# itmo153277/JoshUpscale

Hardware: AMD Instinct MI355X
Metric: frames/sec 480x270->1920x1080 recurrent SR (higher is better)
Workload: dtype bf16

## Files before the change

joshupscale_amd/csrc/tower_kernels.hip:

```cpp
#include "kernel_common.h"

namespace ju {

namespace {

constexpr int kTowerThreads = 256;
constexpr int kTowerWBytes = 9 * 64 * 64 * 2;
constexpr int kTowerTileBytes = 10 * 34 * 128;
constexpr int kTowerLds = kTowerWBytes + 2 * kTowerTileBytes;

__device__ __forceinline__ void glds16(const void *g, void *l) {
	__builtin_amdgcn_global_load_lds((const __attribute__((address_space(1))) void *)g,
	    (__attribute__((address_space(3))) void *)l, 16, 0, 0);
}

struct TowerParams {
	const void *in;
	const void *wgt;
	const float *bias;
	const void *res;
	void *out;
	int H, W, pitch;
	int tilesX, numTiles;
	int relu;
// ... 35 lines not shown
		}
	};

	{
		const unsigned char *wsrc = static_cast<const unsigned char *>(p.wgt);
#pragma unroll
		for (int k = 0; k < (VARIANT == 4 ? 0 : 18); ++k) {
			const int i = wave + 4 * k;
			glds16(wsrc + (size_t)i * 1024 + lane * 16, smW + i * 1024);
		}
	}
	int tile = slot;
	if (tile < p.numTiles) stageTile(tile, 0);

	f32x4 biasv[2][4];
#pragma unroll
	for (int nb = 0; nb < 2; ++nb) {
#pragma unroll
		for (int g = 0; g < 4; ++g) {
			biasv[nb][g] = *reinterpret_cast<const f32x4 *>(p.bias + nb * 32 + 8 * g + 4 * hh);
		}
	}
	asm volatile("s_waitcnt vmcnt(0)" ::: "memory");
	__syncthreads();

	const unsigned ldsBase = static_cast<unsigned>(reinterpret_cast<unsigned long long>(
	    (__attribute__((address_space(3))) unsigned char *)smem));
	const unsigned wAddr = ldsBase + hh * 1024 + px * 16;
	const unsigned wAddrHi = wAddr + 40960;
	const int q0 = (wave * 2) * 34 + px;

	int buf = 0;
	const int stride = perX * 8;
	for (; tile < p.numTiles; tile += stride, buf ^= 1) {
		const int next = tile + stride;
		if (next < p.numTiles) stageTile(next, buf ^ 1);

		const int ty = tile / p.tilesX;
		const int tx = tile - ty * p.tilesX;
		f32x16 acc[2][2];
#pragma unroll
		for (int nb = 0; nb < 2; ++nb) {
#pragma unroll
			for (int g = 0; g < 4; ++g) {
#pragma unroll
				for (int rw = 0; rw < 2; ++rw) {
					acc[nb][rw][4 * g + 0] = biasv[nb][g][0];
					acc[nb][rw][4 * g + 1] = biasv[nb][g][1];
					acc[nb][rw][4 * g + 2] = biasv[nb][g][2];
					acc[nb][rw][4 * g + 3] = biasv[nb][g][3];
				}
			}
		}
		Vec4<T> resv[2][2][4];
		if (VARIANT != 2 && p.res != nullptr) {
			const int gxr = tx * 32 + px;
#pragma unroll
			for (int rw = 0; rw < 2; ++rw) {
				const int gyr = ty * 8 + wave * 2 + rw;
				const T *rp = static_cast<const T *>(p.res) +
				              ((size_t)(gyr + 1) * p.pitch + gxr + 1) * 64 + 4 * hh;
#pragma unroll
				for (int nb = 0; nb < 2; ++nb) {
#pragma unroll
					for (int g = 0; g < 4; ++g) {
						resv[rw][nb][g] = *reinterpret_cast<const Vec4<T> *>(rp + nb * 32 + 8 * g);
					}
				}
			}
		}

		Vec8<T> fa[2][3][2], fb[2][4];
		const unsigned tileAddr = ldsBase + kTowerWBytes + buf * kTowerTileBytes;
		auto issueRead = [&](int m, int set, int idx) {
			const int dx = m >> 2, ks = m & 3;
			constexpr int kind[10] = {0, 1, 0, 1, 0, 0, 1, 0, 0, 1};
			constexpr int sub[10] = {0, 0, 1, 1, 2, 3, 2, 4, 5, 3};
			if (kind[idx] == 0) {
				const int dy = sub[idx] >> 1, nb = sub[idx] & 1;
				const int widx = (dy * 3 + dx) * 4 + ks;
				const int off = widx * 2048 + nb * 512;
				if (off < 65536 - 512) {
					asm volatile("ds_read_b128 %0, %1 offset:%2"
					             : "=v"(fa[set][dy][nb]) : "v"(wAddr), "n"(off));
				} else {
					asm volatile("ds_read_b128 %0, %1 offset:%2"
					             : "=v"(fa[set][dy][nb]) : "v"(wAddrHi), "n"(off - 40960));
				}
			} else {
				const int r = sub[idx];
				const int q = q0 + r * 34 + dx;
				const unsigned a = tileAddr + q * 128 + (((ks * 2 + hh) ^ ((q >> 1) & 7)) << 4);
				asm volatile("ds_read_b128 %0, %1" : "=v"(fb[set][r]) : "v"(a));
			}
		};
		constexpr int needs[12] = {1, 2, 3, -1, 4, 5, 6, -1, 7, 8, 9, -1};
		asm volatile("s_waitcnt lgkmcnt(0)" ::: "memory");
		__builtin_amdgcn_sched_barrier(0);
#pragma unroll
		for (int i = 0; i < (VARIANT == 1 ? 0 : 10); ++i) issueRead(0, 0, i);
#pragma unroll
		for (int m = 0; m < (VARIANT == 1 ? 0 : 12); ++m) {
			const int set = m & 1;
			const bool more = (m + 1 < 12);
#pragma unroll
			for (int k = 0; k < 12; ++k) {
				if (needs[k] >= 0) {
					const int allowed = (9 - needs[k]) + (more ? (k < 10 ? k : 10) : 0);
					if (allowed >= 10) asm volatile("s_waitcnt lgkmcnt(10)" ::: "memory");
					else if (allowed == 9) asm volatile("s_waitcnt lgkmcnt(9)" ::: "memory");
					else if (allowed == 8) asm volatile("s_waitcnt lgkmcnt(8)" ::: "memory");
					else if (allowed == 7) asm volatile("s_waitcnt lgkmcnt(7)" ::: "memory");
					else if (allowed == 6) asm volatile("s_waitcnt lgkmcnt(6)" ::: "memory");
					else if (allowed == 5) asm volatile("s_waitcnt lgkmcnt(5)" ::: "memory");
					else if (allowed == 4) asm volatile("s_waitcnt lgkmcnt(4)" ::: "memory");
					else if (allowed == 3) asm volatile("s_waitcnt lgkmcnt(3)" ::: "memory");
					else if (allowed == 2) asm volatile("s_waitcnt lgkmcnt(2)" ::: "memory");
					else if (allowed == 1) asm volatile("s_waitcnt lgkmcnt(1)" ::: "memory");
					else asm volatile("s_waitcnt lgkmcnt(0)" ::: "memory");
					__builtin_amdgcn_sched_barrier(0);
				}
				const int dy = k >> 2, rw = (k >> 1) & 1, nb = k & 1;
				acc[nb][rw] = mfma32(fa[set][dy][nb], fb[set][rw + dy], acc[nb][rw]);
				if (more && k < 10) issueRead(m + 1, set ^ 1, k);
				__builtin_amdgcn_sched_barrier(0);
			}
		}
		asm volatile("s_waitcnt vmcnt(0)" ::: "memory");
		__syncthreads();
		{
			unsigned char *slice = smT + buf * kTowerTileBytes + wave * 8192;
#pragma unroll
			for (int rw = 0; rw < 2; ++rw) {
				const int pi = rw * 32 + px;
#pragma unroll
				for (int nb = 0; nb < 2; ++nb) {
#pragma unroll
					for (int g = 0; g < 4; ++g) {
						float v[4];
#pragma unroll
						for (int i = 0; i < 4; ++i) v[i] = acc[nb][rw][4 * g + i];
						if (VARIANT != 2 && p.res != nullptr) {
#pragma unroll
							for (int i = 0; i < 4; ++i) v[i] += static_cast<float>(resv[rw][nb][g][i]);
						}
						if (p.relu == 1) {
#pragma unroll
							for (int i = 0; i < 4; ++i) v[i] = fmaxf(v[i], 0.0f);
						} else if (p.relu == 2) {
#pragma unroll
							for (int i = 0; i < 4; ++i) v[i] = leaky(v[i], p.slope);
						}
						Vec4<T> o = {static_cast<T>(v[0]), static_cast<T>(v[1]),
						    static_cast<T>(v[2]), static_cast<T>(v[3])};
						const int c = nb * 4 + g;
						*reinterpret_cast<Vec4<T> *>(
						    slice + pi * 128 + ((c ^ (pi & 7)) << 4) + hh * 8) = o;
					}
				}
			}
			__builtin_amdgcn_fence(__ATOMIC_RELEASE, "wavefront");
			__builtin_amdgcn_wave_barrier();
			__builtin_amdgcn_fence(__ATOMIC_ACQUIRE, "wavefront");
			if (VARIANT != 2) {
				T *outp = static_cast<T *>(p.out);
#pragma unroll
				for (int i = 0; i < 8; ++i) {
					const int pi = i * 8 + (lane >> 3);
					const int c = (lane & 7) ^ (pi & 7);
					typedef unsigned u32x4 __attribute__((ext_vector_type(4)));
					const u32x4 val = *reinterpret_cast<const u32x4 *>(slice + i * 1024 + lane * 16);
					const int gy = ty * 8 + wave * 2 + (pi >> 5);
					const int gxo = tx * 32 + (pi & 31);
					if (gy < p.H && gxo < p.W) {
						*reinterpret_cast<u32x4 *>(
						    outp + ((size_t)(gy + 1) * p.pitch + gxo + 1) * 64 + c * 8) = val;
					}
				}
			} else {
				asm volatile("" ::"v"(acc[0][0]), "v"(acc[1][0]), "v"(acc[0][1]), "v"(acc[1][1]));
			}
		}
		asm volatile("s_waitcnt lgkmcnt(0)" ::: "memory");
		__builtin_amdgcn_s_barrier();
		__builtin_amdgcn_sched_barrier(0);
	}
}

int g_TowerVariant = 0;
int g_ResidentFault = 0;

template <typename T, int VARIANT>
void launchTowerT(const ConvParams &p, hipStream_t stream) {
	auto kern = conv_tower_kernel<T, VARIANT>;
	static std::atomic<std::uint64_t> ldsDone{0};
	ensureDynamicLds(reinterpret_cast<const void *>(kern), kTowerLds, &ldsDone, "tower");
	const int pitch = towerPitch(p.W);
	const size_t origin = towerOrigin(p.W) * 64 * 2;
	TowerParams t{};
	t.in = static_cast<const unsigned char *>(p.in) - origin;
	t.wgt = p.wgt;
	t.bias = p.bias;
	t.res = p.res ? static_cast<const unsigned char *>(p.res) - origin : nullptr;
	t.out = static_cast<unsigned char *>(p.out) - origin;
	t.H = p.H;
	t.W = p.W;
	t.pitch = pitch;
	t.tilesX = (p.W + 31) / 32;
	t.numTiles = t.tilesX * ((p.H + 7) / 8);
	t.relu = p.relu;
	t.slope = p.slope;
	const int grid = ((t.numTiles < 256 ? t.numTiles : 256) + 7) / 8 * 8;
	hipLaunchKernelGGL(kern, dim3(grid), dim3(kTowerThreads), kTowerLds, stream, t);
	hipCheckLaunch("conv_tower");
}

#ifndef JU_TOWER_M16
#define JU_TOWER_M16 1
#endif
#if JU_TOWER_M16
struct TowerAcc {
	f32x4 q[4];
};
__device__ __forceinline__ float accElem(const TowerAcc &a, const int i) { return a.q[i >> 2][i & 3]; }
__device__ __forceinline__ void setAccElem(TowerAcc &a, const int i, const float v) { a.q[i >> 2][i & 3] = v; }
#else
typedef f32x16 TowerAcc;
__device__ __forceinline__ float accElem(const TowerAcc &a, const int i) { return a[i]; }
__device__ __forceinline__ void setAccElem(TowerAcc &a, const int i, const float v) { a[i] = v; }
#endif
constexpr int kResRW = 32;
constexpr int kResMaxRH = 16;
constexpr int kResPitch = kResRW + 2;
constexpr int kResRowBytes = kResPitch * 128;
constexpr int kResBufBytes = (kResMaxRH + 2) * kResRowBytes;
constexpr int kResDummyOff = kResBufBytes;
constexpr int kResOffA = 0;
constexpr int kResOffB = kResBufBytes + 16;
constexpr int kResOffMisc = kResOffB + kResBufBytes + 16;
static_assert(kResRowBytes == 4352, "the ds_read immediates in tower_resident_kernel assume a 4352-byte row");
constexpr int kResLds = kResOffMisc + 64 + 512;
constexpr int kResMailSlots = 4 * 32 * 8;
constexpr unsigned long long kResTimeoutTicks = 20000000ull;
#ifndef JU_PRERUN
#define JU_PRERUN 2
#endif
#ifndef JU_PREBEFORE
#define JU_PREBEFORE 1
#endif
#ifndef JU_FAST_PRERUN
#define JU_FAST_PRERUN 2
#endif

__host__ __device__ inline bool residentFastShape(int rhv, int rwv) {
	if ((rhv & 1) || rwv < 2) return false;
#if JU_TOWER_M16
	if (rwv != 32) return false;
#endif
	const int np2 = rhv >> 1;
	for (int par = 0; par < 2; ++par) {
		const int first = par ? 1 : 2;
		int n = 0;
		for (int k = 0; k < 2; ++k) {
			const int u = first + 2 * k;
			if (u < np2 && 2 * u + 3 <= rhv) n = k + 1;
		}
		const int mine = (np2 - par + 1) >> 1;
		if (n != 2 || (mine != 3 && mine != 4)) return false;
	}
	return true;
}

struct ResidentParams {
	const void *in;
	int inPitch;
	int hasHead;
	void *out;
	const void *weights;
	const float *bias;
	uint4 *mail;
	unsigned *count;
	unsigned *error;
	unsigned long long *debug;
	int H, W, pitch;
	int GX, GY, RH;
	int nLayers;
	float slope;
	const void *tailW1;
	const float *tailB1;
	const void *tailW2;
	const float *tailB2;
	const std::uint8_t *frame;
	std::ptrdiff_t frameStride;
	void *state;
	std::uint8_t *outU8;
	std::ptrdiff_t outStride;
	const unsigned *sums;
};

typedef unsigned long long u64;
typedef __attribute__((address_space(1))) u64 gu64;
typedef __attribute__((address_space(1))) unsigned gu32;

template <typename T, int VARIANT, bool HEAD, bool TAIL = false, bool LEAKY = false, bool FAST = false>
__global__ __launch_bounds__(256, 1) void tower_resident_kernel(ResidentParams p) {
	static_assert(!FAST || ((VARIANT == 0 || VARIANT == 4) && (JU_FAST_PRERUN == 2 || JU_FAST_PRERUN == 3)), "the fast schedule is built for the product only");
	extern __shared__ __attribute__((aligned(16))) unsigned char smem[];
	constexpr bool kNoMfma = VARIANT == 2 || VARIANT == 3;
#ifdef JU_NOXCHG_DEV
	constexpr bool xchg = false;
#else
	constexpr bool xchg = !(VARIANT == 1 || VARIANT == 3);
#endif
	const int tid = threadIdx.x;
	const int wave = tid >> 6;
	const int lane = tid & 63;
	const int px = lane & 31;
	const int hh = lane >> 5;
	const int ch = wave & 1;
	const int rp = wave >> 1;
	int region;
	{
		const int n = gridDim.x, x = blockIdx.x & 7;
		int start = 0;
		for (int y = 0; y < x; ++y) start += (n - y + 7) >> 3;
		region = start + (blockIdx.x >> 3);
	}
	const int gxr = region % p.GX;
	const int gyr = region / p.GX;
	const int x0 = gxr * kResRW;
	const int y0 = gyr * p.RH;
	const int rwv = min(kResRW, p.W - x0);
	const int rhv = min(p.RH, p.H - y0);
	volatile int *failFlag = reinterpret_cast<volatile int *>(smem + kResOffMisc);
	unsigned pubCount[2] = {p.count[region * 2], p.count[region * 2 + 1]};

	const unsigned ldsBase = static_cast<unsigned>(reinterpret_cast<unsigned long long>(
	    (__attribute__((address_space(3))) unsigned char *)smem));

	for (int i = tid; i < kResOffMisc / 16; i += 256) {
		reinterpret_cast<uint4 *>(smem)[i] = make_uint4(0, 0, 0, 0);
	}
	if (tid == 0) *failFlag = 0;
	__syncthreads();

	{
		const T *in = static_cast<const T *>(p.in);
		const int nPix = (rhv + 2) * kResPitch;
		const int nInstr = (nPix + 7) / 8;
		for (int i = wave; i < nInstr; i += 4) {
			const int q = i * 8 + (lane >> 3);
			const int rr = q / kResPitch, cc = q - rr * kResPitch;
			const int c = (lane & 7) ^ ((cc >> 1) & 7);
			const int gy = y0 - 1 + rr, gx = x0 - 1 + cc;
			if (q < nPix && gy >= 0 && gy < p.H && gx >= 0 && gx < p.W) {
				glds16(in + ((size_t)gy * p.inPitch + gx) * 64 + c * 8, smem + kResOffA + i * 1024);
			}
		}
	}

	typedef unsigned u32x4w __attribute__((ext_vector_type(4)));
	const __amdgpu_buffer_rsrc_t wRsrc = __builtin_amdgcn_make_buffer_rsrc(
	    const_cast<void *>(p.weights), 0, p.nLayers * 73728, 0x00020000);
#if JU_TOWER_M16
	const unsigned wLaneOff = (unsigned)((ch * 64 + lane) * 16);
#else
	const unsigned wLaneOff = (unsigned)((hh * 64 + ch * 32 + px) * 16);
#endif
	auto loadWeightFrag = [&](int layer, int f) __attribute__((always_inline)) -> Vec8<T> {
		const u32x4w v = __builtin_amdgcn_raw_buffer_load_b128(wRsrc, wLaneOff, layer * 73728 + f * 2048, 0);
		return __builtin_bit_cast(Vec8<T>, v);
	};
	Vec8<T> wm[12], ws[24];
	auto loadMidWeights = [&](int layer) __attribute__((always_inline)) {
#pragma unroll
		for (int f = 0; f < 36; ++f) {
			if ((f >> 2) % 3 == 1) wm[(f / 12) * 4 + (f & 3)] = loadWeightFrag(layer, f);
		}
	};
	auto loadSideWeights = [&](int layer) __attribute__((always_inline)) {
#pragma unroll
		for (int f = 0; f < 36; ++f) {
			const int dx = (f >> 2) % 3;
			if (dx != 1) ws[(f / 12) * 8 + (dx >> 1) * 4 + (f & 3)] = loadWeightFrag(layer, f);
		}
	};
	loadMidWeights(0);
	loadSideWeights(0);
	const __amdgpu_buffer_rsrc_t biasRsrc = __builtin_amdgcn_make_buffer_rsrc(
	    const_cast<float *>(p.bias), 0, p.nLayers * 256, 0x00020000);
	TowerAcc biasVec;
	auto loadBias = [&](int layer) __attribute__((always_inline)) {
#if JU_TOWER_M16
#pragma unroll
		for (int c16 = 0; c16 < 2; ++c16) {
			const u32x4w v = __builtin_amdgcn_raw_buffer_load_b128(biasRsrc, (unsigned)((ch * 32 + c16 * 16 + 4 * (lane >> 4)) * 4), layer * 256, 0);
#pragma unroll
			for (int i = 0; i < 4; ++i) {
				setAccElem(biasVec, 4 * c16 + i, __uint_as_float(v[i]));
				setAccElem(biasVec, 8 + 4 * c16 + i, __uint_as_float(v[i]));
			}
		}
#else
#pragma unroll
		for (int g = 0; g < 4; ++g) {
			const u32x4w v = __builtin_amdgcn_raw_buffer_load_b128(biasRsrc, (unsigned)((ch * 32 + 4 * hh + 8 * g) * 4), layer * 256, 0);
#pragma unroll
			for (int i = 0; i < 4; ++i) setAccElem(biasVec, 4 * g + i, __uint_as_float(v[i]));
		}
#endif
	};
	loadBias(0);

	unsigned colBase[3], colSwz[3];
#pragma unroll
	for (int dx = 0; dx < 3; ++dx) {
#if JU_TOWER_M16
		const int cq = (lane & 15) + dx;
#else
		const int cq = px + dx;
#endif
		colBase[dx] = cq * 128;
		colSwz[dx] = (cq >> 1) & 7;
	}
	unsigned outsw[4];
#pragma unroll
	for (int g = 0; g < 4; ++g) {
#if JU_TOWER_M16
		const int cq = (g >> 1) * 16 + (lane & 15) + 1;
		outsw[g] = cq * 128 + (((ch * 4 + (g & 1) * 2 + (lane >> 5)) ^ ((cq >> 1) & 7)) << 4) + ((lane >> 4) & 1) * 8;
#else
		const int cq = px + 1;
		outsw[g] = cq * 128 + (((ch * 4 + g) ^ ((cq >> 1) & 7)) << 4) + hh * 8;
#endif
	}

	asm volatile("s_waitcnt vmcnt(0)" ::: "memory");
	__syncthreads();

	u64 prof[8] = {0, 0, 0, 0, 0, 0, 0, 0};
	u64 extraPasses = 0;
	float calibMax = 0.f;
	auto stamp = [&]() __attribute__((always_inline)) -> u64 {
		if constexpr (VARIANT == 4) {
			__builtin_amdgcn_sched_barrier(0);
			u64 t;
			asm volatile("s_memtime %0\n\ts_waitcnt lgkmcnt(0)" : "=s"(t)::"memory");
			__builtin_amdgcn_sched_barrier(0);
			return t;
		} else {
			return 0;
		}
	};
	constexpr int kOrder[12] = {4, 5, 6, 7, 0, 1, 2, 3, 8, 9, 10, 11};
	constexpr bool kPlain = VARIANT == 8;
	constexpr int kPreRun = kPlain ? 0 : FAST ? JU_FAST_PRERUN : JU_PRERUN;
	constexpr int kPreBefore = kPlain ? 0 : JU_PREBEFORE;
	TowerAcc accPre0[2], accPre1[2], accPre2[2];
	static_assert(kPreRun >= 0 && kPreRun <= 3, "at most three interior units per wave");
	Vec8<T> fb[2][4];
	auto issue = [&](unsigned rowAddr, int m, int set, int j) __attribute__((always_inline)) {
#if JU_TOWER_M16
		const int dx = m >> 2, ks32 = (m >> 1) & 1, ph = m & 1;
		const unsigned a = rowAddr + colBase[dx] + (((unsigned)(ks32 * 4 + (lane >> 4)) ^ colSwz[dx]) << 4);
		if (ph) {
			if (j == 0) asm volatile("ds_read_b128 %0, %1 offset:2048" : "=v"(fb[set][0]) : "v"(a));
			else if (j == 1) asm volatile("ds_read_b128 %0, %1 offset:6400" : "=v"(fb[set][1]) : "v"(a));
			else if (j == 2) asm volatile("ds_read_b128 %0, %1 offset:10752" : "=v"(fb[set][2]) : "v"(a));
			else asm volatile("ds_read_b128 %0, %1 offset:15104" : "=v"(fb[set][3]) : "v"(a));
			return;
		}
#else
		const int dx = m >> 2, ks = m & 3;
		const unsigned a = rowAddr + colBase[dx] + (((unsigned)(ks * 2 + hh) ^ colSwz[dx]) << 4);
#endif
		if (j == 0) asm volatile("ds_read_b128 %0, %1" : "=v"(fb[set][0]) : "v"(a));
		else if (j == 1) asm volatile("ds_read_b128 %0, %1 offset:4352" : "=v"(fb[set][1]) : "v"(a));
		else if (j == 2) asm volatile("ds_read_b128 %0, %1 offset:8704" : "=v"(fb[set][2]) : "v"(a));
		else asm volatile("ds_read_b128 %0, %1 offset:13056" : "=v"(fb[set][3]) : "v"(a));
	};
	const int np2 = rhv >> 1;
	const bool mySingle = (rhv & 1) && rp == (np2 & 1);
	const int preFirst = rp ? 1 : 2;
	int nPre = 0;
#pragma unroll
	for (int k = 0; k < kPreRun; ++k) {
		const int u = preFirst + 2 * k;
		if (u < np2 && 2 * u + 3 <= rhv) nPre = k + 1;
	}
	if constexpr (FAST && kPreRun == 3) {
		const int mine = (np2 - rp + 1) >> 1;
		nPre = nPre < mine - 1 ? nPre : mine - 1;
	}
	const int preEnd = preFirst + 2 * nPre;
	auto isPre = [&](int u) __attribute__((always_inline)) { return u >= preFirst && u < preEnd; };
	auto nextWhole = [&](int u) __attribute__((always_inline)) {
		int v = u + 2;
		if (isPre(v)) v = preEnd;
		return v < np2 ? v : -1;
	};
	const int firstWhole = isPre(rp) ? (preEnd < np2 ? preEnd : -1) : (rp < np2 ? rp : -1);
	const bool streamsInUnit = (firstWhole >= 0 || mySingle) && !kNoMfma && !kPlain;
	constexpr bool kDefer = FAST;
	const bool deferShape = residentFastShape(rhv, rwv);
	if constexpr (FAST) {
		if (!deferShape) {
			if (tid == 0) __hip_atomic_store((gu32 *)p.error, 0x6f0u, __ATOMIC_RELAXED, __HIP_MEMORY_SCOPE_SYSTEM);
			return;
		}
	}

#if JU_TOWER_M16
	const bool validLo = (lane & 15) < rwv, validHi = 16 + (lane & 15) < rwv;
	auto groupValid = [&](const int g) __attribute__((always_inline)) { return FAST || ((g >> 1) ? validHi : validLo); };
#else
	const bool lanesValid = px < rwv;
	auto groupValid = [&](const int) __attribute__((always_inline)) { return lanesValid; };
#endif
	typedef unsigned u32x4 __attribute__((ext_vector_type(4)));
	const __amdgpu_buffer_rsrc_t mailRsrc = __builtin_amdgcn_make_buffer_rsrc(
	    (void *)p.mail, 0, (int)((size_t)p.GX * p.GY * 2 * (LEAKY ? 2 : 1) * kResMailSlots * 16), 0x00020000);
	constexpr int kSc1 = 16;
	Vec4<T> rvNext[2][4];
	auto epiValue = [&](auto resTag, const TowerAcc &a, const int g, const Vec4<T> &rv, float(&v)[4]) __attribute__((always_inline)) {
#pragma unroll
		for (int i = 0; i < 4; ++i) v[i] = accElem(a, 4 * g + i);
		if constexpr (decltype(resTag)::value) {
#pragma unroll
			for (int i = 0; i < 4; ++i) v[i] += static_cast<float>(rv[i]);
		}
		if constexpr (VARIANT == 5 && !LEAKY) {
			if (groupValid(g)) {
#pragma unroll
				for (int i = 0; i < 4; ++i) calibMax = fmaxf(calibMax, v[i]);
			}
		}
	};
	auto epiStore = [&](auto outTag, const int row, const int g, float(&v)[4]) __attribute__((always_inline)) {
		constexpr int outOff = decltype(outTag)::value;
		if constexpr (LEAKY) {
#pragma unroll
			for (int i = 0; i < 4; ++i) v[i] = fmaxf(v[i], v[i] * p.slope);
			if constexpr (VARIANT == 5) {
#pragma unroll
				for (int i = 0; i < 4; ++i) calibMax = fmaxf(calibMax, fabsf(v[i]));
			}
			*reinterpret_cast<Vec4<T> *>(smem + outOff + row * kResRowBytes + outsw[g]) = pack4<T>(v[0], v[1], v[2], v[3]);
		} else {
			*reinterpret_cast<Vec4<T> *>(smem + outOff + row * kResRowBytes + outsw[g]) =
			    reluPacked<T>(pack4<T>(v[0], v[1], v[2], v[3]));
		}
	};
	auto unitSeg = [&](auto rowsTag, auto kindTag, auto resTag, auto inTag, auto outTag, TowerAcc(&acc)[2],
	                   const int layer, const int unit, const bool primed, const int nextUnit,
	                   const bool nextFinish, auto streamTag, auto defTag, TowerAcc(&dacc)[2], const int dunit,
	                   auto epiTag) __attribute__((always_inline)) {
		constexpr bool streamNext = decltype(streamTag)::value;
		constexpr bool DEF = decltype(defTag)::value;
		constexpr bool EPI = decltype(epiTag)::value;
		constexpr int ROWS = decltype(rowsTag)::value;
		constexpr int KIND = decltype(kindTag)::value;
		constexpr bool residual = decltype(resTag)::value;
		constexpr int inOff = decltype(inTag)::value;
		constexpr int outOff = decltype(outTag)::value;
		constexpr int P0 = KIND == 1 ? 4 : 0;
		constexpr int P1 = KIND == 0 ? 4 : 12;
		const u64 tu0 = stamp();
		constexpr int NR = ROWS + 2;
		constexpr int NM = 3 * ROWS;
		const int ra = 1 + 2 * unit;
		if constexpr (KIND != 1 && kNoMfma) {
#pragma unroll
			for (int r = 0; r < ROWS; ++r) acc[r] = biasVec;
		}
		unsigned rowAddr = ldsBase + inOff + (2 * unit) * kResRowBytes;
		asm volatile("" : "+v"(rowAddr));
		constexpr bool kFetchRes = !EPI && residual && KIND != 0;
		const int dra = 1 + 2 * dunit;
		const TowerAcc dacc0 = dacc[0], dacc1 = dacc[1];
		float dv[4];
		unsigned dlo = 0, dhi = 0;
		auto defSlot = [&](const int pos, const int k, const int part = -1) __attribute__((always_inline)) {
					if constexpr (DEF) {
						const int j = pos - P0;
						if (j < 8) {
							const int r = j >> 2, g = j & 3;
							if (k < 5 && part == 1) {
							} else if (k < 4) {
								dv[k] = accElem(r ? dacc1 : dacc0, 4 * g + k);
								if constexpr (residual) {
									dv[k] += static_cast<float>(rvNext[r][g][k]);
									asm volatile("" : "+v"(dv[k]));
								}
								if constexpr (LEAKY) {
									const float t = dv[k] * p.slope;
									asm volatile("v_max_f32 %0, %1, %2" : "=v"(dv[k]) : "v"(dv[k]), "v"(t));
								}
							} else if (k == 4) {
								const Vec4<T> pk = pack4<T>(dv[0], dv[1], dv[2], dv[3]);
								typedef unsigned u32x2d __attribute__((ext_vector_type(2)));
								const u32x2d w = __builtin_bit_cast(u32x2d, pk);
								dlo = w[0];
								dhi = w[1];
								asm volatile("" : "+v"(dlo), "+v"(dhi));
							} else {
								typedef unsigned u32x2d __attribute__((ext_vector_type(2)));
								if (part != 1) {
									const Vec4<T> pk = __builtin_bit_cast(Vec4<T>, u32x2d{dlo, dhi});
									const u32x2d w = __builtin_bit_cast(u32x2d, LEAKY ? pk : reluPacked<T>(pk));
									dlo = w[0];
									dhi = w[1];
									if (part == 0) asm volatile("" : "+v"(dlo), "+v"(dhi));
								}
								if (part != 0) {
									const Vec4<T> o = __builtin_bit_cast(Vec4<T>, u32x2d{dlo, dhi});
									if (groupValid(g)) *reinterpret_cast<Vec4<T> *>(smem + outOff + (dra + r) * kResRowBytes + outsw[g]) = o;
								}
							}
						}
					}
		};
// ... 287 lines not shown
		if (valid) pubValid |= 1u << it;
		if (kLean && !valid) pubLds[it] = 0u;
	}
	const unsigned pubBase = (unsigned)(region * 2 * kSlots) * 16u + (unsigned)tid * 16u;
	unsigned sweepSrc[NS];
	unsigned sweepLds[NS];
	unsigned sweepValid = 0;
#pragma unroll
	for (int it = 0; it < NS; ++it) {
		int nx = gxr, ny = gyr, strip, se, rr, cc, cs;
		bool valid;
		if (it < NS - 1) {
			const int idx = it * 256 + tid;
			const int hp = idx >> CSH;
			cs = idx & (CPP - 1);
			int side = hp >> 5, e = hp & 31;
			if (kCompact && it >= ROWITS) {
				const int j = (it - ROWITS) * 256 + tid;
				side = 2 + j / COLPT;
				e = (j / CPP) & 15;
			}
			if (side < 2) {
				ny += side == 0 ? -1 : 1;
				strip = side == 0 ? 1 : 0;
				rr = side == 0 ? 0 : rhv + 1;
				se = e;
				cc = e + 1;
				valid = e < rwv;
			} else {
				nx += side == 2 ? -1 : 1;
				strip = side == 2 ? 3 : 2;
				se = e;
				rr = e + 1;
				cc = side == 2 ? 0 : rwv + 1;
				valid = e < rhv;
			}
		} else {
			const int k = tid >> CSH;
			cs = tid & (CPP - 1);
			const bool up = k < 2, left = (k & 1) == 0;
			ny += up ? -1 : 1;
			nx += left ? -1 : 1;
			strip = up ? 1 : 0;
			se = left ? kResRW - 1 : 0;
			rr = up ? 0 : rhv + 1;
			cc = left ? 0 : rwv + 1;
			valid = tid < 4 * CPP;
		}
		const int c = LEAKY ? cs >> 1 : cs, half = LEAKY ? (cs & 1) * 8 : 0;
		valid = valid && nx >= 0 && nx < p.GX && ny >= 0 && ny < p.GY;
		const int nreg = valid ? ny * p.GX + nx : region;
		sweepSrc[it] = (unsigned)((nreg * 2) * kSlots + (strip * 32 + se) * CPP + cs) * 16u;
		sweepLds[it] = (unsigned)(rr * kResRowBytes + cc * 128 + ((c ^ ((cc >> 1) & 7)) << 4) + half);
		if (valid) sweepValid |= 1u << it;
		if (kLean && !valid) {
			sweepSrc[it] = (unsigned)((region * 2) * kSlots + (tid & (CPP - 1))) * 16u;
			sweepLds[it] = (unsigned)kResDummyOff;
		}
	}
	constexpr unsigned kParityBytes = kSlots * 16u;
	auto publish = [&](auto offTag, int layer) __attribute__((always_inline)) {
		constexpr int off = decltype(offTag)::value;
		const int ppar = (layer + 1) & 1;
		pubCount[ppar] += 1u;
		const unsigned soff = ppar ? kParityBytes : 0u;
		if constexpr (LEAKY) {
			typedef unsigned u32x2 __attribute__((ext_vector_type(2)));
			const unsigned tg = pubCount[ppar] << 16;
			u32x2 v[NP];
#pragma unroll
			for (int it = 0; it < NP; ++it) v[it] = *reinterpret_cast<const u32x2 *>(smem + off + pubLds[it]);
#pragma unroll
			for (int it = 0; it < NP; ++it) {
				if (kLean || (pubValid >> it & 1u)) {
					const u32x4 d = {(v[it][0] & 0xffffu) | tg, (v[it][0] >> 16) | tg, (v[it][1] & 0xffffu) | tg,
					    (v[it][1] >> 16) | tg};
					__builtin_amdgcn_raw_buffer_store_b128(d, mailRsrc, kCompact ? pubOff[it] : pubBase + it * 4096, soff, kSc1);
				}
			}
		} else {
			const unsigned tm = epochMask(ppar);
			u32x4 v[NP];
#pragma unroll
			for (int it = 0; it < NP; ++it) v[it] = *reinterpret_cast<const u32x4 *>(smem + off + pubLds[it]);
#pragma unroll
			for (int it = 0; it < NP; ++it) {
				if constexpr (kCompact) {
					__builtin_amdgcn_raw_buffer_store_b128(v[it] | tm, mailRsrc, pubOff[it], soff, kSc1);
				} else if (pubValid >> it & 1u) {
					__builtin_amdgcn_raw_buffer_store_b128((v[it] & 0x7fff7fffu) | tm, mailRsrc,
					    pubBase + it * 4096, soff, kSc1);
				}
			}
		}
		asm volatile("s_nop 1" ::: "memory");
	};
	auto fillHalo = [&](auto offTag, int layer, auto &&behindFirstPass) __attribute__((always_inline)) -> bool {
		constexpr int off = decltype(offTag)::value;
		u64 t0 = 0;
		const int par = (layer + 1) & 1;
		const unsigned tm = LEAKY ? (pubCount[par] & 0xffffu) : epochMask(par);
		const unsigned soff = par ? kParityBytes : 0u;
		unsigned pending = sweepValid;
		u32x4 hvFirst[NS];
		auto loadPassTo = [&](u32x4(&hv)[NS]) __attribute__((always_inline)) {
#pragma unroll
			for (int it = 0; it < NS; ++it) {
				hv[it] = __builtin_amdgcn_raw_buffer_load_b128(mailRsrc, sweepSrc[it], soff, kSc1);
			}
		};
		auto checkPassOf = [&](const u32x4(&hv)[NS]) __attribute__((always_inline)) {
#pragma unroll
			for (int it = 0; it < NS; ++it) {
				if constexpr (LEAKY) {
					typedef unsigned u32x2 __attribute__((ext_vector_type(2)));
					const u32x4 tg = hv[it] >> 16;
					const bool ok = tg[0] == tm && tg[1] == tm && tg[2] == tm && tg[3] == tm;
					if ((pending >> it & 1u) && ok) {
						*reinterpret_cast<u32x2 *>(smem + off + sweepLds[it]) =
						    u32x2{(hv[it][0] & 0xffffu) | (hv[it][1] << 16), (hv[it][2] & 0xffffu) | (hv[it][3] << 16)};
						pending &= ~(1u << it);
					}
				} else {
					const u32x4 tg = hv[it] & 0x80008000u;
					const bool ok = tg[0] == tm && tg[1] == tm && tg[2] == tm && tg[3] == tm;
					if ((pending >> it & 1u) && ok) {
						*reinterpret_cast<u32x4 *>(smem + off + sweepLds[it]) = hv[it] & 0x7fff7fffu;
						pending &= ~(1u << it);
					}
				}
			}
		};
		auto checkPassFast = [&](const u32x4(&hv)[NS]) __attribute__((always_inline)) {
			unsigned bad = 0;
#pragma unroll
			for (int it = 0; it < NS; ++it) {
				if constexpr (LEAKY) {
					typedef unsigned u32x2 __attribute__((ext_vector_type(2)));
					const u32x4 x = hv[it] ^ (tm << 16);
					bad |= x[0] | x[1] | x[2] | x[3];
					*reinterpret_cast<u32x2 *>(smem + off + sweepLds[it]) = u32x2{(x[0] & 0xffffu) | (x[1] << 16), (x[2] & 0xffffu) | (x[3] << 16)};
				} else {
					const u32x4 x = hv[it] ^ tm;
					bad |= x[0] | x[1] | x[2] | x[3];
					*reinterpret_cast<u32x4 *>(smem + off + sweepLds[it]) = x;
				}
			}
			pending = bad & (LEAKY ? 0xffff0000u : 0x80008000u);
		};
		auto loadPass = [&]() __attribute__((always_inline)) { loadPassTo(hvFirst); };
		auto checkPass = [&]() __attribute__((always_inline)) {
			if constexpr (kLean) checkPassFast(hvFirst);
			else checkPassOf(hvFirst);
		};
		loadPass();
		__builtin_amdgcn_sched_barrier(0);
		behindFirstPass();
		__builtin_amdgcn_sched_barrier(0);
#ifdef JU_TOWER_FILLPROF
		const u64 fp0 = stamp();
#endif
		if constexpr (FAST) {
			u32x4 hvSecond[NS];
			loadPassTo(hvSecond);
			__builtin_amdgcn_sched_barrier(0);
			if constexpr (kLean) {
				checkPassFast(hvFirst);
				if (__any(pending != 0)) {
					checkPassFast(hvSecond);
					if constexpr (VARIANT == 4) extraPasses += 1;
				}
			} else {
				checkPassOf(hvFirst);
				if (__any(pending != 0)) {
					checkPassOf(hvSecond);
					if constexpr (VARIANT == 4) extraPasses += 1;
				}
			}
		} else {
			checkPass();
		}
#ifdef JU_TOWER_FILLPROF
		const u64 fp1 = stamp();
#endif
		while (__any(pending != 0)) {
			const u64 now = __builtin_amdgcn_s_memrealtime();
			if (t0 == 0) t0 = now;
			if (now - t0 > kResTimeoutTicks) {
				if (pending != 0) {
					*failFlag = 1;
					__hip_atomic_store((gu32 *)p.error, 0x700u + (unsigned)layer, __ATOMIC_RELAXED,
					    __HIP_MEMORY_SCOPE_SYSTEM);
				}
				break;
			}
			__builtin_amdgcn_s_sleep(1);
			loadPass();
			checkPass();
			if constexpr (VARIANT == 4) extraPasses += 1;
		}
#ifdef JU_TOWER_FILLPROF
		const u64 fp2 = stamp();
#endif
		__syncthreads();
#ifdef JU_TOWER_FILLPROF
		const u64 fp3 = stamp();
		prof[1] += fp1 - fp0;
		prof[3] += fp2 - fp1;
		prof[4] += fp3 - fp2;
#endif
		return *failFlag == 0;
	};

	const int L = p.nLayers;
	auto layerStep = [&](auto resTag, auto parTag, const int i) __attribute__((always_inline)) -> bool {
		constexpr int PAR = decltype(parTag)::value;
		using InT = std::integral_constant<int, PAR ? kResOffB : kResOffA>;
		using OutT = std::integral_constant<int, PAR ? kResOffA : kResOffB>;
		const bool more = i + 1 < L;
		const u64 t0 = stamp();
		finishLayer(resTag, InT{}, OutT{}, i, more && streamsInUnit);
		if constexpr (VARIANT == 5) {
			float m = calibMax;
#pragma unroll
			for (int off = 32; off > 0; off >>= 1) m = fmaxf(m, __shfl_xor(m, off));
			if (lane == 0) atomicMax(reinterpret_cast<unsigned *>(p.debug) + i, __float_as_uint(m));
			calibMax = 0.f;
		}
		const u64 t1 = stamp();
		__syncthreads();
		const u64 t2 = stamp();
		if (more && xchg) publish(OutT{}, i);
		const bool primePre = more && nPre > 0 && !kNoMfma;
		if (primePre) {
			const unsigned na = ldsBase + OutT::value + (2 * preFirst) * kResRowBytes;
#pragma unroll
			for (int j = 0; j < 4; ++j) issue(na, kOrder[0], 0, j);
			__builtin_amdgcn_sched_barrier(0);
		}
		const u64 t3 = stamp();
		if (more && !streamsInUnit) {
			loadBias(i + 1);
			loadMidWeights(i + 1);
			loadSideWeights(i + 1);
		}
		const u64 t4 = stamp();
		if (more && xchg) {
			using Z = std::integral_constant<int, 0>;
			using Split = std::integral_constant<int, kPreBefore>;
			using N = std::integral_constant<int, kPreRun>;
			preRun(OutT{}, InT{}, Z{}, Split{}, i + 1, primePre);
			const bool okFill = fillHalo(OutT{}, i, [&]() __attribute__((always_inline)) {
				preRun(OutT{}, InT{}, Split{}, N{}, i + 1, primePre);
			});
			if (!okFill) return false;
		} else {
			if (more) preRun(OutT{}, InT{}, std::integral_constant<int, 0>{}, std::integral_constant<int, kPreRun>{}, i + 1, primePre);
			__syncthreads();
		}
		const u64 t5 = stamp();
		prof[0] += t5 - t4;
#ifndef JU_TOWER_FILLPROF
		prof[1] += (VARIANT == 4 && FAST) ? extraPasses * 1000 : t4 - t3;
#endif
		extraPasses = 0;
		prof[2] += t1 - t0;
#if !defined(JU_TOWER_SEGPROF) && !defined(JU_TOWER_FILLPROF)
		prof[3] += t2 - t1;
		prof[4] += t3 - t2;
#endif
		return true;
	};
	using No = std::false_type;
	using Yes = std::true_type;
	using P0 = std::integral_constant<int, 0>;
	using P1 = std::integral_constant<int, 1>;
	preRun(std::integral_constant<int, kResOffA>{}, std::integral_constant<int, kResOffB>{}, std::integral_constant<int, 0>{},
	    std::integral_constant<int, kPreRun>{}, 0, false);
	if (HEAD) {
		if (!layerStep(No{}, P0{}, 0)) return;
		for (int i = 1; i + 1 < L; i += 2) {
			if (!layerStep(No{}, P1{}, i)) return;
			if (!layerStep(Yes{}, P0{}, i + 1)) return;
		}
	} else {
		for (int i = 0; i + 1 < L; i += 2) {
			if (!layerStep(No{}, P0{}, i)) return;
			if (!layerStep(Yes{}, P1{}, i + 1)) return;
		}
	}
	const int finalOff = (L & 1) ? kResOffB : kResOffA;
	if (tid == 0 && xchg) {
		p.count[region * 2] = pubCount[0];
		p.count[region * 2 + 1] = pubCount[1];
	}
	if constexpr (VARIANT == 4) {
		if (lane == 0 && p.debug != nullptr) {
			for (int k = 0; k < 8; ++k) p.debug[(region * 4 + wave) * 8 + k] = prof[k];
		}
	}

	if constexpr (TAIL) {
		const int scratchOff = finalOff == kResOffA ? kResOffB : kResOffA;
		static_assert(kTailLdsW1 + 4 * (kTailLdsMid / 4 + kTailLdsRow + kTailLdsU8 / 4) <= kResBufBytes,
		    "tail scratch must fit one activation buffer");
		unsigned char *smW = smem + scratchOff;
		unsigned char *waveBase = smW + kTailLdsW1 + wave * (kTailLdsMid / 4 + kTailLdsRow + kTailLdsU8 / 4);
		unsigned char *smMid = waveBase;
		unsigned char *smState = waveBase + kTailLdsMid / 4;
		unsigned char *smU8 = smState + kTailLdsRow;
		{
			const uint4 *src = reinterpret_cast<const uint4 *>(p.tailW1);
			uint4 *dst = reinterpret_cast<uint4 *>(smW);
#pragma unroll
			for (int k = 0; k < kTailLdsW1 / 16 / 256; ++k) dst[tid + k * 256] = src[tid + k * 256];
		}
		Vec8<T> a2[2];
		a2[0] = reinterpret_cast<const Vec8<T> *>(p.tailW2)[lane];
		a2[1] = reinterpret_cast<const Vec8<T> *>(p.tailW2)[64 + lane];
		const float b2v[3] = {p.tailB2[0], p.tailB2[1], p.tailB2[2]};
		const TailRowArgs args{p.tailB1, p.frame, p.frameStride, p.state, p.outU8, p.outStride, p.H, p.W, -1.0f};
		const float bright = brightnessOf(p.sums, 1.0f / static_cast<float>(p.H * p.W));
		__syncthreads();
		for (int r = wave; r < rhv; r += 4) {
			const unsigned char *rowBase = smem + finalOff + (r + 1) * kResRowBytes;
			const auto fetchB = [&](int ks) {
				const int cc = px + 1;
				return *reinterpret_cast<const Vec8<T> *>(
				    rowBase + cc * 128 + (((ks * 2 + hh) ^ ((cc >> 1) & 7)) << 4));
			};
			tailRow<T>(fetchB, smW, smMid, smState, smU8, a2, b2v, args, bright, x0, y0 + r, lane);
		}
		return;
	}

	{
		T *out = static_cast<T *>(p.out);
		for (int i = tid; i < rhv * kResRW * 8; i += 256) {
			const int c = i & 7;
			const int pxl = (i >> 3) % kResRW;
			const int row = (i >> 3) / kResRW;
			if (pxl < rwv) {
				const int rr = row + 1, cc = pxl + 1;
				const uint4 v = *reinterpret_cast<const uint4 *>(
				    smem + finalOff + rr * kResRowBytes + cc * 128 + ((c ^ ((cc >> 1) & 7)) << 4));
				*reinterpret_cast<uint4 *>(
				    out + ((size_t)(y0 + rr) * p.pitch + x0 + cc) * 64 + c * 8) = v;
			}
		}
	}
}

template <typename T, int VARIANT, bool HEAD, bool TAIL = false, bool LEAKY = false, bool FAST = false>
void launchResidentT(const ResidentParams &p, hipStream_t stream) {
	auto kern = tower_resident_kernel<T, VARIANT, HEAD, TAIL, LEAKY, FAST>;
	static std::atomic<std::uint64_t> ldsDone{0};
	ensureDynamicLds(reinterpret_cast<const void *>(kern), kResLds, &ldsDone, "resident tower");
	const int grid = p.GX * p.GY - (g_ResidentFault < p.GX * p.GY ? g_ResidentFault : 0);
	hipLaunchKernelGGL(kern, dim3(grid), dim3(256), kResLds, stream, p);
	hipCheckLaunch("tower_resident");
}

}

void launchConvTower(DType dt, const ConvParams &p, hipStream_t stream) {
	const int pitch = towerPitch(p.W);
	const bool fits = p.taps == 9 && p.cin == 64 && p.cout == 64 && !p.outHead && p.nb == 2 &&
	                  p.inPitch == pitch && p.outPitch == pitch &&
	                  (p.res == nullptr || p.resPitch == pitch);
	if (!fits) {
		launchConv(dt, p, stream);
		return;
	}
	if (dt == kF16) {
		launchTowerT<f16, 0>(p, stream);
		return;
	}
	switch (g_TowerVariant) {
	case 1: launchTowerT<bf16, 1>(p, stream); break;
	case 2: launchTowerT<bf16, 2>(p, stream); break;
	case 3: launchTowerT<bf16, 3>(p, stream); break;
	case 4: launchTowerT<bf16, 4>(p, stream); break;
	default: launchTowerT<bf16, 0>(p, stream); break;
	}
}

bool residentTowerM16() { return JU_TOWER_M16 != 0; }
void setTowerVariant(int v) { g_TowerVariant = v; }
static std::atomic<int> g_TowerFast{[] { const char *e = devSwitch(Dev::TowerFast); return (e != nullptr && e[0] == '0') ? 0 : 1; }()};
void setResidentTowerFast(int on) { g_TowerFast = on ? 1 : 0; }
bool residentTowerFast() { return g_TowerFast.load() != 0; }
int towerVariant() { return g_TowerVariant; }
void setResidentFault(int n) { g_ResidentFault = n; }
int residentFaultForTests() { return g_ResidentFault; }

bool residentTowerGeometry(int H, int W, int numCUs, int *GX, int *GY, int *RH) {
	const int gx = (W + kResRW - 1) / kResRW;
	const int gy = (H + kResMaxRH - 1) / kResMaxRH;
	if (gx * gy > numCUs) return false;
	*GX = gx;
	*GY = gy;
	*RH = (H + gy - 1) / gy;
	return true;
}

bool residentTowerFastGeometry(int H, int W, int GX, int GY, int RH) {
	const int lastH = H - (GY - 1) * RH, lastW = W - (GX - 1) * kResRW;
	return residentFastShape(RH, kResRW) && residentFastShape(lastH, kResRW) && residentFastShape(RH, lastW) &&
	       residentFastShape(lastH, lastW);
}

std::size_t residentMailboxBytes(int GX, int GY, bool leaky) {
	return static_cast<std::size_t>(GX) * GY * 2 * kResMailSlots * 16 * (leaky ? 2 : 1);
}

void launchResidentTower(DType dt, const ResidentTowerParams &q, hipStream_t stream) {
	ResidentParams p{};
	const std::size_t origin = towerOrigin(q.W) * 64 * 2;
	p.in = q.in;
	p.inPitch = q.inPitch ? q.inPitch : q.W;
	p.hasHead = q.hasHead;
	p.out = static_cast<unsigned char *>(q.out) - origin;
	p.weights = q.weights;
	p.bias = q.bias;
	p.mail = static_cast<uint4 *>(q.mailbox);
	p.count = q.counters;
	p.debug = static_cast<unsigned long long *>(q.debug);
	p.error = q.error;
	p.H = q.H;
	p.W = q.W;
	p.pitch = towerPitch(q.W);
	p.GX = q.GX;
	p.GY = q.GY;
	p.RH = q.RH;
	p.nLayers = q.nLayers;
	p.slope = q.slope;
	p.tailW1 = q.tailW1;
	p.tailB1 = q.tailB1;
	p.tailW2 = q.tailW2;
	p.tailB2 = q.tailB2;
	p.frame = q.frame;
	p.frameStride = q.frameStride;
	p.state = q.state;
	p.outU8 = q.outU8;
	p.outStride = q.outStride;
	p.sums = q.sums;
	if ((p.nLayers & 1) != (p.hasHead ? 1 : 0)) {
		throw std::invalid_argument("resident tower: layer count must be 2*blocks (+1 with a head)");
	}
	const bool fast = residentTowerFast() && residentTowerFastGeometry(p.H, p.W, p.GX, p.GY, p.RH);
#ifdef JU_TOWER_DEV
	if (q.leaky || dt == kF16 || !p.hasHead) throw std::invalid_argument("resident tower: developer build");
	if (p.tailW1 != nullptr) {
		if (fast) launchResidentT<bf16, 0, true, true, false, true>(p, stream);
		else launchResidentT<bf16, 0, true, true>(p, stream);
	} else if (g_TowerVariant == 8) launchResidentT<bf16, 8, true>(p, stream);
	else if (g_TowerVariant == 4) {
		if (fast) launchResidentT<bf16, 4, true, false, false, true>(p, stream);
		else launchResidentT<bf16, 4, true>(p, stream);
	} else if (fast) launchResidentT<bf16, 0, true, false, false, true>(p, stream);
	else launchResidentT<bf16, 0, true>(p, stream);
	return;
#else
	if (q.leaky) {
		if (!(q.slope >= 0.0f && q.slope <= 1.0f)) throw std::invalid_argument("resident tower: negative slope outside [0, 1]");
		if (p.tailW1 != nullptr) throw std::invalid_argument("resident tower: the fused tail is built for ReLU models");
		if (!p.hasHead) {
			if (fast) {
				if (dt == kF16) launchResidentT<f16, 0, false, false, true, true>(p, stream);
				else launchResidentT<bf16, 0, false, false, true, true>(p, stream);
			} else {
				if (dt == kF16) launchResidentT<f16, 0, false, false, true>(p, stream);
				else launchResidentT<bf16, 0, false, false, true>(p, stream);
			}
		} else if (g_TowerVariant == 8) {
			if (dt == kF16) launchResidentT<f16, 8, true, false, true>(p, stream);
			else launchResidentT<bf16, 8, true, false, true>(p, stream);
		} else if (g_TowerVariant == 5 && dt == kBF16) {
			(void)hipMemsetAsync(p.debug, 0, static_cast<std::size_t>(p.nLayers) * sizeof(unsigned), stream);
			launchResidentT<bf16, 5, true, false, true>(p, stream);
		} else if (fast && g_TowerVariant == 0) {
			if (dt == kF16) launchResidentT<f16, 0, true, false, true, true>(p, stream);
			else launchResidentT<bf16, 0, true, false, true, true>(p, stream);
		} else {
			if (dt == kF16) launchResidentT<f16, 0, true, false, true>(p, stream);
			else launchResidentT<bf16, 0, true, false, true>(p, stream);
		}
		return;
	}
	if (!p.hasHead) {
		if (fast) {
			if (dt == kF16) launchResidentT<f16, 0, false, false, false, true>(p, stream);
			else launchResidentT<bf16, 0, false, false, false, true>(p, stream);
		} else {
			if (dt == kF16) launchResidentT<f16, 0, false>(p, stream);
			else launchResidentT<bf16, 0, false>(p, stream);
		}
		return;
	}
	if (p.tailW1 != nullptr) {
		if (fast) {
			if (dt == kF16) launchResidentT<f16, 0, true, true, false, true>(p, stream);
			else launchResidentT<bf16, 0, true, true, false, true>(p, stream);
		} else {
			if (dt == kF16) launchResidentT<f16, 0, true, true>(p, stream);
			else launchResidentT<bf16, 0, true, true>(p, stream);
		}
		return;
	}
	if (dt == kF16) {
		if (g_TowerVariant == 8) launchResidentT<f16, 8, true>(p, stream);
		else if (fast) launchResidentT<f16, 0, true, false, false, true>(p, stream);
		else launchResidentT<f16, 0, true>(p, stream);
		return;
	}
	switch (g_TowerVariant) {
	case 8: launchResidentT<bf16, 8, true>(p, stream); break;
	case 1: launchResidentT<bf16, 1, true>(p, stream); break;
	case 2: launchResidentT<bf16, 2, true>(p, stream); break;
	case 3: launchResidentT<bf16, 3, true>(p, stream); break;
	case 4:
		if (fast) launchResidentT<bf16, 4, true, false, false, true>(p, stream);
		else launchResidentT<bf16, 4, true>(p, stream);
		break;
	case 5:
		(void)hipMemsetAsync(p.debug, 0, static_cast<std::size_t>(p.nLayers) * sizeof(unsigned), stream);
		launchResidentT<bf16, 5, true>(p, stream);
		break;
	default:
		if (fast) launchResidentT<bf16, 0, true, false, false, true>(p, stream);
		else launchResidentT<bf16, 0, true>(p, stream);
		break;
	}
#endif
}


}
```

Measured before the change: 2192.

## Keep resident tail weights in registers and overlap stage-2 MFMA with VALU

Replaces the tail of the resident tower kernel with a per-wave routine. It holds the first tail conv weights and biases in registers instead of copying them to LDS behind a block-wide barrier. It prefetches the low-res frame pixels before the stage-1 MFMAs and software-pipelines the stage-2 MFMA of the next block with the VALU epilogue of the current one, using wave-level fences instead of block syncs. The cost is much higher register pressure in a launch_bounds(256,1) kernel, with possible spills.

```diff
diff --git a/joshupscale_amd/csrc/tower_kernels.hip b/joshupscale_amd/csrc/tower_kernels.hip
--- a/joshupscale_amd/csrc/tower_kernels.hip
+++ b/joshupscale_amd/csrc/tower_kernels.hip
@@ -361,6 +361,197 @@
 typedef __attribute__((address_space(1))) u64 gu64;
 typedef __attribute__((address_space(1))) unsigned gu32;
 
+constexpr int kResTailWave = kTailLdsMid / 4 + kTailLdsRow + kTailLdsU8 / 4;
+static_assert(4 * kResTailWave <= kResBufBytes, "tail scratch must fit one activation buffer");
+
+template <typename T>
+struct ResidentTail {
+	Vec8<T> a1[4][4];
+	f32x16 b1[4];
+	Vec8<T> a2[2];
+	float b2v[3];
+	float bright;
+
+	__device__ __forceinline__ void load(const ResidentParams &p, const int lane) {
+		const int px = lane & 31, hh = lane >> 5;
+		const unsigned char *w1 = static_cast<const unsigned char *>(p.tailW1);
+#pragma unroll
+		for (int ks = 0; ks < 4; ++ks) {
+#pragma unroll
+			for (int nb = 0; nb < 4; ++nb) {
+				a1[ks][nb] = *reinterpret_cast<const Vec8<T> *>(
+				    w1 + (nb >> 1) * (64 * 64 * 2) + (((ks * 2 + hh) * 64 + (nb & 1) * 32 + px) << 4));
+			}
+		}
+#pragma unroll
+		for (int nb = 0; nb < 4; ++nb) {
+#pragma unroll
+			for (int g = 0; g < 4; ++g) {
+				const f32x4 b = *reinterpret_cast<const f32x4 *>(p.tailB1 + nb * 32 + 8 * g + 4 * hh);
+#pragma unroll
+				for (int i = 0; i < 4; ++i) b1[nb][4 * g + i] = b[i];
+			}
+		}
+		a2[0] = reinterpret_cast<const Vec8<T> *>(p.tailW2)[lane];
+		a2[1] = reinterpret_cast<const Vec8<T> *>(p.tailW2)[64 + lane];
+#pragma unroll
+		for (int c = 0; c < 3; ++c) b2v[c] = p.tailB2[c];
+		bright = brightnessOf(p.sums, 1.0f / static_cast<float>(p.H * p.W));
+	}
+};
+
+struct TailLr {
+	unsigned v[2][2];
+};
+
+template <typename T>
+__device__ __forceinline__ TailLr tailLoadLr(const ResidentParams &p, const int tx0, const int h, const int lane) {
+	const int w = tx0 + (lane & 31);
+	const int hc = min(h, p.H - 1), wc = min(w, p.W - 1);
+	const int h1 = min(hc + 1, p.H - 1), w1 = min(wc + 1, p.W - 1);
+	TailLr lr;
+#pragma unroll
+	for (int yy = 0; yy < 2; ++yy) {
+#pragma unroll
+		for (int xx = 0; xx < 2; ++xx) {
+			lr.v[yy][xx] = *reinterpret_cast<const unsigned *>(p.frame + (yy ? h1 : hc) * p.frameStride + (xx ? w1 : wc) * 4);
+		}
+	}
+	return lr;
+}
+
+template <typename T>
+__device__ __forceinline__ void tailStage1Slice(const ResidentTail<T> &tr, const unsigned char *rowBase, const int ks,
+    f32x16 (&acc)[4], const int lane) {
+	const int cc = (lane & 31) + 1;
+	const Vec8<T> b = *reinterpret_cast<const Vec8<T> *>(rowBase + cc * 128 + (((ks * 2 + (lane >> 5)) ^ ((cc >> 1) & 7)) << 4));
+#pragma unroll
+	for (int nb = 0; nb < 4; ++nb) acc[nb] = mfma32(tr.a1[ks][nb], b, acc[nb]);
+}
+
+template <typename T>
+__device__ __forceinline__ void tailWriteMid(const f32x16 (&acc)[4], unsigned char *smMid, const int lane) {
+	const int px = lane & 31, hh = lane >> 5;
+#pragma unroll
+	for (int nb = 0; nb < 4; ++nb) {
+#pragma unroll
+		for (int g = 0; g < 4; ++g) {
+			const Vec4<T> o = reluPacked<T>(pack4<T>(acc[nb][4 * g + 0], acc[nb][4 * g + 1], acc[nb][4 * g + 2], acc[nb][4 * g + 3]));
+			*reinterpret_cast<Vec4<T> *>(smMid + nb * 2048 + px * 64 + ((g ^ ((px >> 2) & 3)) << 4) + hh * 8) = o;
+		}
+	}
+}
+
+template <typename T>
+__device__ __forceinline__ f32x16 tailStage2Mfma(const ResidentTail<T> &tr, const int nb, const unsigned char *smMid, const int lane) {
+	const int px = lane & 31, hh = lane >> 5;
+	f32x16 d = {0.f, 0.f, 0.f, 0.f, 0.f, 0.f, 0.f, 0.f, 0.f, 0.f, 0.f, 0.f, 0.f, 0.f, 0.f, 0.f};
+#pragma unroll
+	for (int ks = 0; ks < 2; ++ks) {
+		const int c = ks * 2 + hh;
+		const Vec8<T> b = *reinterpret_cast<const Vec8<T> *>(smMid + nb * 2048 + px * 64 + ((c ^ ((px >> 2) & 3)) << 4));
+		d = mfma32(tr.a2[ks], b, d);
+	}
+	return d;
+}
+
+template <typename T>
+__device__ __forceinline__ void tailStage2Valu(const ResidentTail<T> &tr, const int nb, const f32x16 &d,
+    unsigned char *smState, unsigned char *smU8, const float (&lrv)[2][2][3], const int lane) {
+	const int px = lane & 31, hh = lane >> 5;
+	const int a = nb >> 1, bb = nb & 1;
+#pragma unroll
+	for (int g2 = 0; g2 < 2; ++g2) {
+		const int yq = 2 * a + g2, xq = 2 * bb + hh;
+		const float fy = yq * 0.25f, fx = xq * 0.25f;
+		Vec4<f16> st;
+		unsigned packed = 0;
+#pragma unroll
+		for (int c = 0; c < 3; ++c) {
+			const float top = lrv[0][0][c] + (lrv[0][1][c] - lrv[0][0][c]) * fx;
+			const float bot = lrv[1][0][c] + (lrv[1][1][c] - lrv[1][0][c]) * fx;
+			const float skip = top + (bot - top) * fy;
+			float r = fastTanh(d[4 * g2 + c] + tr.b2v[c]) + skip;
+			r = fminf(fmaxf(r, -0.5f), 0.5f);
+			st[c] = static_cast<f16>(r - tr.bright);
+			const unsigned u = static_cast<unsigned>((r + 0.5f) * 255.0f);
+			packed |= (u & 0xff) << (8 * c);
+		}
+		st[3] = static_cast<f16>(0.f);
+		const int xcol = 4 * px + xq;
+		*reinterpret_cast<Vec4<f16> *>(smState + yq * 1024 + xcol * 8) = st;
+		*reinterpret_cast<unsigned *>(smU8 + yq * 512 + xcol * 4) = packed;
+	}
+}
+
+template <typename T>
+__device__ __forceinline__ void tailWaveSync() {
+	__builtin_amdgcn_fence(__ATOMIC_RELEASE, "wavefront");
+	__builtin_amdgcn_wave_barrier();
+	__builtin_amdgcn_fence(__ATOMIC_ACQUIRE, "wavefront");
+}
+
+template <typename T>
+__device__ __forceinline__ void tailStoreRow(const ResidentParams &p, const unsigned char *smState, const unsigned char *smU8,
+    const int tx0, const int h, const int lane) {
+	const int WW = 4 * p.W;
+	const int nValidPx = min(128, 4 * (p.W - tx0));
+	f16 *stateOut = static_cast<f16 *>(p.state);
+#pragma unroll
+	for (int yq = 0; yq < 4; ++yq) {
+		const int Y = 4 * h + yq;
+		if (2 * lane < nValidPx) {
+			const uint4 v = *reinterpret_cast<const uint4 *>(smState + yq * 1024 + lane * 16);
+			*reinterpret_cast<uint4 *>(stateOut + ((size_t)Y * WW + 4 * tx0 + 2 * lane) * 4) = v;
+			const uint2 u = *reinterpret_cast<const uint2 *>(smU8 + yq * 512 + lane * 8);
+			*reinterpret_cast<uint2 *>(p.outU8 + Y * p.outStride + (4 * tx0 + 2 * lane) * 4) = u;
+		}
+	}
+}
+
+template <typename T>
+__device__ __forceinline__ void residentTailRows(const ResidentParams &p, const unsigned char *fin, unsigned char *scratch,
+    const int x0, const int y0, const int rhv, const int wave, const int lane) {
+	if (wave >= rhv) return;
+	ResidentTail<T> tr;
+	tr.load(p, lane);
+	unsigned char *smMid = scratch + wave * kResTailWave;
+	unsigned char *smState = smMid + kTailLdsMid / 4;
+	unsigned char *smU8 = smState + kTailLdsRow;
+	for (int r = wave; r < rhv; r += 4) {
+		const TailLr lr = tailLoadLr<T>(p, x0, y0 + r, lane);
+		f32x16 acc[4];
+#pragma unroll
+		for (int nb = 0; nb < 4; ++nb) acc[nb] = tr.b1[nb];
+#pragma unroll
+		for (int ks = 0; ks < 4; ++ks) tailStage1Slice<T>(tr, fin + (r + 1) * kResRowBytes, ks, acc, lane);
+		tailWriteMid<T>(acc, smMid, lane);
+		tailWaveSync<T>();
+		float lrv[2][2][3];
+#pragma unroll
+		for (int yy = 0; yy < 2; ++yy) {
+#pragma unroll
+			for (int xx = 0; xx < 2; ++xx) {
+				const unsigned v = lr.v[yy][xx];
+				lrv[yy][xx][0] = preprocessU8(v & 0xff);
+				lrv[yy][xx][1] = preprocessU8((v >> 8) & 0xff);
+				lrv[yy][xx][2] = preprocessU8((v >> 16) & 0xff);
+			}
+		}
+		f32x16 d = tailStage2Mfma<T>(tr, 0, smMid, lane);
+#pragma unroll
+		for (int nb = 0; nb < 4; ++nb) {
+			f32x16 dn = d;
+			if (nb < 3) dn = tailStage2Mfma<T>(tr, nb + 1, smMid, lane);
+			tailStage2Valu<T>(tr, nb, d, smState, smU8, lrv, lane);
+			d = dn;
+		}
+		tailWaveSync<T>();
+		tailStoreRow<T>(p, smState, smU8, x0, y0 + r, lane);
+		tailWaveSync<T>();
+	}
+}
+
 template <typename T, int VARIANT, bool HEAD, bool TAIL = false, bool LEAKY = false, bool FAST = false>
 __global__ __launch_bounds__(256, 1) void tower_resident_kernel(ResidentParams p) {
 	static_assert(!FAST || ((VARIANT == 0 || VARIANT == 4) && (JU_FAST_PRERUN == 2 || JU_FAST_PRERUN == 3)), "the fast schedule is built for the product only");
@@ -374,8 +565,8 @@
 	const int tid = threadIdx.x;
 	const int wave = tid >> 6;
 	const int lane = tid & 63;
-	const int px = lane & 31;
-	const int hh = lane >> 5;
+	[[maybe_unused]] const int px = lane & 31;
+	[[maybe_unused]] const int hh = lane >> 5;
 	const int ch = wave & 1;
 	const int rp = wave >> 1;
 	int region;
@@ -1269,35 +1460,7 @@
 
 	if constexpr (TAIL) {
 		const int scratchOff = finalOff == kResOffA ? kResOffB : kResOffA;
-		static_assert(kTailLdsW1 + 4 * (kTailLdsMid / 4 + kTailLdsRow + kTailLdsU8 / 4) <= kResBufBytes,
-		    "tail scratch must fit one activation buffer");
-		unsigned char *smW = smem + scratchOff;
-		unsigned char *waveBase = smW + kTailLdsW1 + wave * (kTailLdsMid / 4 + kTailLdsRow + kTailLdsU8 / 4);
-		unsigned char *smMid = waveBase;
-		unsigned char *smState = waveBase + kTailLdsMid / 4;
-		unsigned char *smU8 = smState + kTailLdsRow;
-		{
-			const uint4 *src = reinterpret_cast<const uint4 *>(p.tailW1);
-			uint4 *dst = reinterpret_cast<uint4 *>(smW);
-#pragma unroll
-			for (int k = 0; k < kTailLdsW1 / 16 / 256; ++k) dst[tid + k * 256] = src[tid + k * 256];
-		}
-		Vec8<T> a2[2];
-		a2[0] = reinterpret_cast<const Vec8<T> *>(p.tailW2)[lane];
-		a2[1] = reinterpret_cast<const Vec8<T> *>(p.tailW2)[64 + lane];
-		const float b2v[3] = {p.tailB2[0], p.tailB2[1], p.tailB2[2]};
-		const TailRowArgs args{p.tailB1, p.frame, p.frameStride, p.state, p.outU8, p.outStride, p.H, p.W, -1.0f};
-		const float bright = brightnessOf(p.sums, 1.0f / static_cast<float>(p.H * p.W));
-		__syncthreads();
-		for (int r = wave; r < rhv; r += 4) {
-			const unsigned char *rowBase = smem + finalOff + (r + 1) * kResRowBytes;
-			const auto fetchB = [&](int ks) {
-				const int cc = px + 1;
-				return *reinterpret_cast<const Vec8<T> *>(
-				    rowBase + cc * 128 + (((ks * 2 + hh) ^ ((cc >> 1) & 7)) << 4));
-			};
-			tailRow<T>(fetchB, smW, smMid, smState, smU8, a2, b2v, args, bright, x0, y0 + r, lane);
-		}
+		residentTailRows<T>(p, smem + finalOff, smem + scratchOff, x0, y0, rhv, wave, lane);
 		return;
 	}
 
```

Measured after the change: 2206, median of 6. About the same (+0.6%).
